# thrill/thrill

Measured on NVIDIA H100. Metric: sort_keys_per_s, higher is better.
Workload: dtype u64

## Files before the change

### thrill_b200/csrc/tg_partition.cuh

```cuda
#pragma once
#include "tg_common.cuh"

namespace tgp {

constexpr int RADIX_BITS = 8;
constexpr int RADIX = 1 << RADIX_BITS;

constexpr u32 FLAG_PARTIAL = 1u << 30;
constexpr u32 FLAG_INCL = 2u << 30;
constexpr u32 VALUE_MASK = (1u << 30) - 1;

template <int WORDS> struct ItemT;
template <> struct ItemT<1> { typedef u64 type; };
template <> struct ItemT<2> { typedef ulonglong2 type; };

__device__ __forceinline__ u64 item_word(const u64& v, int) { return v; }
__device__ __forceinline__ u64 item_word(const ulonglong2& v, int w) { return w ? v.y : v.x; }

struct RadixDigit {
    int word, shift;
    u32 flip;
    static constexpr bool kStoreDigit = false;
    static constexpr bool kHasDrop = false;
    static constexpr int kScratch = 0;
    __device__ __forceinline__ void init() {}
    template <class Item>
    __device__ __forceinline__ u32 operator()(const Item& v, u32) const {
        return ((u32)(item_word(v, word) >> shift) & (RADIX - 1)) ^ flip;
    }
};

__device__ __forceinline__ u32 match_digit8(u32 d) {
    u32 peers;
    asm volatile(
        "{\n"
        ".reg .pred p0, p1, p2, p3, p4, p5, p6, p7;\n"
        ".reg .b32 m0, m1, m2, m3, m4, m5, m6, m7, t;\n"
        "and.b32 t, %1, 1;   setp.ne.u32 p0, t, 0;\n"
        "and.b32 t, %1, 2;   setp.ne.u32 p1, t, 0;\n"
        "and.b32 t, %1, 4;   setp.ne.u32 p2, t, 0;\n"
        "and.b32 t, %1, 8;   setp.ne.u32 p3, t, 0;\n"
        "and.b32 t, %1, 16;  setp.ne.u32 p4, t, 0;\n"
        "and.b32 t, %1, 32;  setp.ne.u32 p5, t, 0;\n"
        "and.b32 t, %1, 64;  setp.ne.u32 p6, t, 0;\n"
        "and.b32 t, %1, 128; setp.ne.u32 p7, t, 0;\n"
        "vote.sync.ballot.b32 m0, p0, 0xffffffff;\n"
        "vote.sync.ballot.b32 m1, p1, 0xffffffff;\n"
        "vote.sync.ballot.b32 m2, p2, 0xffffffff;\n"
        "vote.sync.ballot.b32 m3, p3, 0xffffffff;\n"
        "vote.sync.ballot.b32 m4, p4, 0xffffffff;\n"
        "vote.sync.ballot.b32 m5, p5, 0xffffffff;\n"
        "vote.sync.ballot.b32 m6, p6, 0xffffffff;\n"
        "vote.sync.ballot.b32 m7, p7, 0xffffffff;\n"
        "@!p0 not.b32 m0, m0;\n"
        "@!p1 not.b32 m1, m1;\n"
        "@!p2 not.b32 m2, m2;\n"
        "@!p3 not.b32 m3, m3;\n"
        "@!p4 not.b32 m4, m4;\n"
        "@!p5 not.b32 m5, m5;\n"
        "@!p6 not.b32 m6, m6;\n"
        "@!p7 not.b32 m7, m7;\n"
        "lop3.b32 t, m0, m1, m2, 0x80;\n"
        "lop3.b32 t, t, m3, m4, 0x80;\n"
        "lop3.b32 t, t, m5, m6, 0x80;\n"
        "and.b32 %0, t, m7;\n"
        "}\n"
        : "=r"(peers)
        : "r"(d));
    return peers;
}

constexpr int PEER_MAX = 32;
template <int WORDS, bool STORE = true, bool PEER = false, int SCRATCH = 0>
struct PartCfg {
    static constexpr int THREADS = 512;
    static constexpr int MIN_BLOCKS = 1;
    static constexpr int ITEM_BYTES = 8 * WORDS;
    static constexpr int ITEMS = 32 / WORDS;
    static constexpr int TILE = THREADS * ITEMS;
    static constexpr int HALF = TILE / 2;
    static constexpr int TILE_BYTES = TILE * ITEM_BYTES;
    static constexpr int NWARPS = THREADS / 32;
    static constexpr int BUF_BYTES = TILE_BYTES + (WORDS == 1 ? 16 : 0);
    static constexpr int SMEM = BUF_BYTES + HALF * ITEM_BYTES + NWARPS * RADIX * (int)sizeof(unsigned short) + RADIX * 4 + 64 + 16 + (STORE ? HALF : 0) + (PEER ? PEER_MAX * 8 : 0) + SCRATCH + 128;
    static_assert(SMEM <= 227 * 1024, "partition pass: shared memory of one CTA");
};
constexpr u32 TILE_GROUP = 8;

static __global__ void scan_hist_kernel(const u32* __restrict__ ghist, u32* __restrict__ gbase, u32* __restrict__ skip,
                                 int npass, u32 n) {
    __shared__ u32 warp_tot[RADIX / 32];
    const int d = threadIdx.x;
    for (int p = 0; p < npass; ++p) {
        u32 c = ghist[p * RADIX + d];
        u32 incl = c;
#pragma unroll
        for (int o = 1; o < 32; o <<= 1) {
            u32 t = __shfl_up_sync(0xffffffffu, incl, o);
            if ((d & 31) >= o) incl += t;
        }
        if ((d & 31) == 31) warp_tot[d >> 5] = incl;
        __syncthreads();
        u32 add = 0;
        for (int w = 0; w < (d >> 5); ++w) add += warp_tot[w];
        gbase[p * RADIX + d] = add + incl - c;
        u32 full = __syncthreads_or(c == n);
        if (d == 0 && skip) skip[p] = full ? 1u : 0u;
        __syncthreads();
    }
}

__device__ __forceinline__ u32 lds_u32(u32 addr) {
    u32 v;
    asm volatile("ld.shared.u32 %0, [%1];" : "=r"(v) : "r"(addr) : "memory");
    return v;
}
__device__ __forceinline__ void sts_u32(u32 addr, u32 v) { asm volatile("st.shared.u32 [%0], %1;" ::"r"(addr), "r"(v) : "memory"); }
typedef unsigned short cnt_t;
__device__ __forceinline__ u32 lds_cnt(u32 addr) {
    u32 v;
    asm volatile("ld.shared.u16 %0, [%1];" : "=r"(v) : "r"(addr) : "memory");
    return v;
}
__device__ __forceinline__ void sts_cnt(u32 addr, u32 v) { asm volatile("st.shared.u16 [%0], %1;" ::"r"(addr), "r"(v) : "memory"); }

template <bool FULL, bool STORE, int ITEMS, class Item, class DigitFn>
__device__ __forceinline__ void rank_rows(const Item (&key)[ITEMS], u32 (&rank)[ITEMS], const DigitFn& fn, u32 whist_w,
                                          u32 pos0, u32 tile_base, u32 tile_valid, u32 lt) {
#pragma unroll
    for (int i = 0; i < ITEMS; ++i) {
        const u32 p = pos0 + i * 32;
        u32 d = fn(key[i], tile_base + p);
        if (!FULL && p >= tile_valid) d = RADIX - 1;
        const u32 a = whist_w + d * (u32)sizeof(cnt_t);
        const u32 old = lds_cnt(a);
        const u32 peers = match_digit8(d);
        const u32 below = peers & lt;
        if (below == 0) sts_cnt(a, old + __popc(peers));
        rank[i] = old + __popc(below);
        if (STORE) rank[i] |= d << 16;
        __syncwarp();
    }
}

template <bool STORE, int ITEMS, class Item, class DigitFn>
__device__ __forceinline__ void rank_rows_unstable(const Item (&key)[ITEMS], u32 (&rank)[ITEMS], const DigitFn& fn, u32 whist_w,
                                                   u32 pos0, u32 tile_base) {
#pragma unroll
    for (int i = 0; i < ITEMS; ++i) {
        const u32 d = fn(key[i], tile_base + pos0 + i * 32);
        const u32 sh = (d & 1u) << 4;
        u32 old;
        asm volatile("atom.shared.add.u32 %0, [%1], %2;" : "=r"(old) : "r"(whist_w + (d >> 1) * 4u), "r"(1u << sh) : "memory");
        rank[i] = (old >> sh) & 0xffffu;
        if (STORE) rank[i] |= d << 16;
    }
}

struct SegList {
    const uint4* tiles;
    const u32* segbase;
    u32 num_tiles;
    const u32* num_tiles_dev;
};
__device__ __forceinline__ u32 seg_num_tiles(const SegList& sl) { return sl.num_tiles_dev ? __ldg(sl.num_tiles_dev) : sl.num_tiles; }

template <int WORDS, class DigitFn, bool SEG, bool PEER, bool UNSTABLE>
__global__ void __launch_bounds__(PartCfg<WORDS>::THREADS, PartCfg<WORDS>::MIN_BLOCKS)
partition_kernel(const typename ItemT<WORDS>::type* __restrict__ in, typename ItemT<WORDS>::type* __restrict__ out,
                 u32 n, const DigitFn fn_param, const u32* __restrict__ gbase, u32* __restrict__ status, const SegList sl,
                 typename ItemT<WORDS>::type* const* __restrict__ dbase) {
    typedef typename ItemT<WORDS>::type Item;
    typedef PartCfg<WORDS, DigitFn::kStoreDigit, PEER, DigitFn::kScratch> C;
    constexpr int THREADS = C::THREADS, ITEMS = C::ITEMS, TILE = C::TILE, HALF = C::HALF, NWARPS = C::NWARPS;
    constexpr int LB = 8;
    static_assert(TILE_GROUP <= (u32)LB, "a group member reaches past its group's first tile with one batch");
    static_assert(THREADS >= RADIX, "one thread per digit in the scan phases");

    extern __shared__ __align__(1024) unsigned char smem_raw[];
    Item* const buf = reinterpret_cast<Item*>(smem_raw);
    Item* const xbuf = reinterpret_cast<Item*>(smem_raw + C::BUF_BYTES);
    cnt_t* const whist = reinterpret_cast<cnt_t*>(xbuf + HALF);
    u32* const goff = reinterpret_cast<u32*>(whist + NWARPS * RADIX);
    u32* const warp_tot = goff + RADIX;
    u64* const mbar = reinterpret_cast<u64*>(warp_tot + 16);
    unsigned char* const dig = reinterpret_cast<unsigned char*>(mbar + 2);
    Item** const dptr = reinterpret_cast<Item**>(dig + (DigitFn::kStoreDigit ? HALF : 0));
    unsigned char* const fscratch = reinterpret_cast<unsigned char*>(dptr + (PEER ? PEER_MAX : 0));

    DigitFn fn = fn_param;
    fn.init();
    if constexpr (DigitFn::kScratch > 0) fn.init_shared(fscratch, (int)threadIdx.x, THREADS);
    const int tid = threadIdx.x, lane = tid & 31, warp = tid >> 5;
    const u32 num_tiles = SEG ? seg_num_tiles(sl) : (n + TILE - 1) / TILE;
    const u32 lt = lanemask_lt();
    cnt_t* const whist_w = whist + warp * RADIX;
    const u32 whist_w_a = smem_u32(whist_w);
    const u32 wbase = warp * 32 * ITEMS;

    struct TileInfo { u32 start, len, row, idx, seg; };
    auto tile_info = [&](u32 j) -> TileInfo {
        TileInfo ti;
        if (SEG) {
            const uint4 d = __ldg(&sl.tiles[j]);
            ti.start = d.x; ti.len = d.y; ti.row = d.z; ti.idx = d.w & 0xfffffu; ti.seg = d.w >> 20;
        }
        else {
            ti.start = j * TILE;
            ti.len = (n - ti.start < (u32)TILE) ? n - ti.start : (u32)TILE;
            ti.row = j; ti.idx = j; ti.seg = 0;
        }
        return ti;
    };
    auto tma_shift = [&](const TileInfo& ti) -> u32 { return WORDS == 1 ? (ti.start & 1u) : 0u; };
    auto tma_ok = [&](const TileInfo& ti) -> bool {
        if (ti.len != (u32)TILE) return false;
        return tma_shift(ti) == 0 || (size_t)ti.start + TILE + 1 <= n;
    };

    if (tid == 0) {
        mbar_init(&mbar[0], 1);
        mbar_fence_init();
    }
    if (PEER && tid < PEER_MAX) dptr[tid] = dbase[tid];
    __syncthreads();

    u32 j = blockIdx.x;
    TileInfo tnext = tile_info(j < num_tiles ? j : 0);
    TileInfo tnext2 = tile_info(j + gridDim.x < num_tiles ? j + gridDim.x : 0);
    if (j < num_tiles) {
        const TileInfo t0 = tnext;
        if (tid == 0 && tma_ok(t0)) {
            const u32 sh = tma_shift(t0), bytes = C::TILE_BYTES + 16 * sh;
            mbar_expect_tx(&mbar[0], bytes);
            bulk_g2s(buf, in + (t0.start - sh), bytes, &mbar[0]);
        }
    }
    u32 phase = 0;

    for (; j < num_tiles; j += gridDim.x) {
        const TileInfo ti = tnext;
        if (j + gridDim.x < num_tiles) tnext = tnext2;
        if (SEG ? (j + 2 * gridDim.x < num_tiles) : true) tnext2 = tile_info(j + 2 * gridDim.x);
        const u32 tile_base = ti.start;
        const bool full_tile = ti.len == (u32)TILE;
        const u32 tile_valid = ti.len;
        const bool by_tma = tma_ok(ti);
        const u32* const gb = SEG ? sl.segbase + (size_t)ti.seg * RADIX : gbase;

#pragma unroll
        for (int i = 0; i < RADIX / 64; ++i) reinterpret_cast<u32*>(whist_w)[i * 32 + lane] = 0;

        Item key[ITEMS];
        u32 rank[ITEMS];
        if (by_tma) {
            mbar_wait(&mbar[0], phase);
            phase ^= 1u;
            const Item* src = buf + tma_shift(ti) + wbase + lane;
#pragma unroll
            for (int i = 0; i < ITEMS; ++i) key[i] = src[i * 32];
        }
        else if (full_tile) {
            const Item* src = in + tile_base + wbase + lane;
#pragma unroll
            for (int i = 0; i < ITEMS; ++i) key[i] = src[i * 32];
        }
        else {
#pragma unroll
            for (int i = 0; i < ITEMS; ++i) {
                u32 p = wbase + i * 32 + lane;
                if (p < tile_valid) key[i] = in[(size_t)tile_base + p];
            }
        }
        __syncwarp();

        if (full_tile && UNSTABLE) rank_rows_unstable<DigitFn::kStoreDigit>(key, rank, fn, whist_w_a, wbase + lane, tile_base);
        else if (full_tile) rank_rows<true, DigitFn::kStoreDigit>(key, rank, fn, whist_w_a, wbase + lane, tile_base, tile_valid, lt);
        else rank_rows<false, true>(key, rank, fn, whist_w_a, wbase + lane, tile_base, tile_valid, lt);
        __syncthreads();

        if (tid == 0 && j + gridDim.x < num_tiles) {
            const TileInfo tn = tnext;
            if (tma_ok(tn)) {
                const u32 sh = tma_shift(tn), bytes = C::TILE_BYTES + 16 * sh;
                fence_proxy_async();
                mbar_expect_tx(&mbar[0], bytes);
                bulk_g2s(buf, in + (tn.start - sh), bytes, &mbar[0]);
            }
        }

        u32 count = 0, my_start = 0;
        u32 lbv[SEG ? 1 : LB];
        const u32 my_gb = tid < RADIX ? __ldg(&gb[tid]) : 0u;
        u32* const my_status = status + (size_t)ti.row * RADIX + tid;
        if (tid < RADIX) {
#pragma unroll
            for (int w = 0; w < NWARPS; ++w) count += whist[w * RADIX + tid];
            u32 pub = count;
            if (!full_tile && tid == RADIX - 1) pub -= (u32)TILE - tile_valid;
            st_relaxed_u32(my_status, pub | (ti.idx == 0 ? FLAG_INCL : FLAG_PARTIAL));
            if (SEG) {
                lbv[0] = ti.idx > 0 ? ld_relaxed_u32(my_status - RADIX) : FLAG_INCL;
            }
            else {
#pragma unroll
                for (int k = 0; k < LB; ++k)
                    lbv[k] = ((u32)(k + 1) <= ti.idx) ? ld_relaxed_u32(my_status - (size_t)(k + 1) * RADIX) : FLAG_INCL;
            }
            u32 incl = count;
#pragma unroll
            for (int o = 1; o < 32; o <<= 1) {
                u32 v = __shfl_up_sync(0xffffffffu, incl, o);
                if (lane >= o) incl += v;
            }
            if (lane == 31) warp_tot[warp] = incl;
            my_start = incl - count;
        }
        __syncthreads();
        if (tid < RADIX) {
            for (int w = 0; w < warp; ++w) my_start += warp_tot[w];
            u32 off = my_start;
#pragma unroll
            for (int w = 0; w < NWARPS; ++w) {
                u32 c = whist[w * RADIX + tid];
                whist[w * RADIX + tid] = (cnt_t)off;
                off += c;
            }
        }
        __syncthreads();

#pragma unroll
        for (int r = 0; r < 2; ++r) {
            if (full_tile && !DigitFn::kStoreDigit) {
#pragma unroll
                for (int i = 0; i < ITEMS; ++i) {
                    u32 d = fn(key[i], 0);
                    u32 q = lds_cnt(whist_w_a + d * (u32)sizeof(cnt_t)) + rank[i] - (u32)(r * HALF);
                    if (q < (u32)HALF) xbuf[q] = key[i];
                }
            }
            else {
#pragma unroll
                for (int i = 0; i < ITEMS; ++i) {
                    u32 d = rank[i] >> 16;
                    u32 q = lds_cnt(whist_w_a + d * (u32)sizeof(cnt_t)) + (rank[i] & 0xffffu) - (u32)(r * HALF);
                    if (q < (u32)HALF) {
                        xbuf[q] = key[i];
                        if (DigitFn::kStoreDigit) dig[q] = (unsigned char)d;
                    }
                }
            }

            if (r == 0 && tid < RADIX) {
                u32 excl = 0;
                if (ti.idx > 0) {
                    u32 back = 1;
                    bool done = false;
                    u32 v[LB];
                    if (SEG) {
                        if (lbv[0] & FLAG_INCL) { excl = lbv[0] & VALUE_MASK; done = true; }
                        else {
                            v[0] = lbv[0];
#pragma unroll
                            for (int k = 1; k < LB; ++k)
                                v[k] = (back + k <= ti.idx) ? ld_relaxed_u32(my_status - (size_t)(back + k) * RADIX) : FLAG_INCL;
                        }
                    }
                    else {
#pragma unroll
                        for (int k = 0; k < LB; ++k) v[k] = lbv[k];
                    }
                    while (!done) {
                        bool stalled = false;
#pragma unroll
                        for (int k = 0; k < LB; ++k) {
                            if (!done && !stalled) {
                                if (v[k] & FLAG_INCL) { excl += v[k] & VALUE_MASK; done = true; }
                                else if (v[k] & FLAG_PARTIAL) { excl += v[k] & VALUE_MASK; back++; }
                                else stalled = true;
                            }
                        }
                        if (done) break;
#pragma unroll
                        for (int k = 0; k < LB; ++k)
                            v[k] = (back + k <= ti.idx) ? ld_relaxed_u32(my_status - (size_t)(back + k) * RADIX) : FLAG_INCL;
                    }
                    u32 pub = count;
                    if (!full_tile && tid == RADIX - 1) pub -= (u32)TILE - tile_valid;
                    st_relaxed_u32(my_status, (excl + pub) | FLAG_INCL);
                }
                goff[tid] = my_gb + excl - my_start;
            }
            __syncthreads();

            {
                const Item* const bufp = xbuf + tid;
                const u32 q0 = (u32)(r * HALF) + tid;
                if (full_tile) {
#pragma unroll
                    for (int i = 0; i < HALF / THREADS; ++i) {
                        Item v = bufp[i * THREADS];
                        u32 d = DigitFn::kStoreDigit ? (u32)dig[i * THREADS + tid] : fn(v, 0);
                        if (DigitFn::kHasDrop && d == RADIX - 1) continue;
                        if (PEER) dptr[d][goff[d] + q0 + (u32)(i * THREADS)] = v;
                        else out[goff[d] + q0 + (u32)(i * THREADS)] = v;
                    }
                }
                else {
#pragma unroll
                    for (int i = 0; i < HALF / THREADS; ++i) {
                        if (q0 + (u32)(i * THREADS) < tile_valid) {
                            Item v = bufp[i * THREADS];
                            u32 d = DigitFn::kStoreDigit ? (u32)dig[i * THREADS + tid] : fn(v, 0);
                            if (DigitFn::kHasDrop && d == RADIX - 1) continue;
                            if (PEER) dptr[d][goff[d] + q0 + (u32)(i * THREADS)] = v;
                            else out[goff[d] + q0 + (u32)(i * THREADS)] = v;
                        }
                    }
                }
            }
            __syncthreads();
        }
    }
}

template <int WORDS>
__global__ void copy_items_kernel(const typename ItemT<WORDS>::type* __restrict__ in,
                                  typename ItemT<WORDS>::type* __restrict__ out, size_t n) {
    size_t stride = (size_t)gridDim.x * blockDim.x;
    for (size_t i = (size_t)blockIdx.x * blockDim.x + threadIdx.x; i < n; i += stride) out[i] = in[i];
}

template <int WORDS>
constexpr u32 tile_items() { return (u32)PartCfg<WORDS>::TILE; }
template <int WORDS>
constexpr u32 num_tiles_for(size_t n) { return (u32)((n + tile_items<WORDS>() - 1) / tile_items<WORDS>()); }

template <int WORDS, class DigitFn, bool SEG, bool PEER = false, bool UNSTABLE = false>
int launch_partition_v(tg_ctx* ctx, const void* in, void* out, u32 n, const DigitFn& fn, const u32* gbase, u32* status,
                       const SegList& sl, typename ItemT<WORDS>::type* const* dbase = nullptr) {
    typedef typename ItemT<WORDS>::type Item;
    typedef PartCfg<WORDS, DigitFn::kStoreDigit, PEER, DigitFn::kScratch> C;
    auto kern = partition_kernel<WORDS, DigitFn, SEG, PEER, UNSTABLE>;
    int ctas_per_sm = 0;
    auto it = ctx->kernel_cfg.find((const void*)kern);
    if (it != ctx->kernel_cfg.end()) ctas_per_sm = it->second;
    else {
        TG_CUDA(ctx, cudaFuncSetAttribute(kern, cudaFuncAttributeMaxDynamicSharedMemorySize, C::SMEM));
        TG_CUDA(ctx, cudaOccupancyMaxActiveBlocksPerMultiprocessor(&ctas_per_sm, kern, C::THREADS, C::SMEM));
        if (ctas_per_sm < 1) return tg_set_error(ctx, TG_ERR_CUDA, "partition kernel does not fit on an SM");
        if (ctas_per_sm > C::MIN_BLOCKS) ctas_per_sm = C::MIN_BLOCKS;
        ctx->kernel_cfg[(const void*)kern] = ctas_per_sm;
    }
    u32 num_tiles = SEG ? sl.num_tiles : (n + C::TILE - 1) / C::TILE;
    if (num_tiles == 0) return TG_OK;
    int grid = ctx->sm_count * ctas_per_sm;
    if (grid > (int)num_tiles) grid = (int)num_tiles;
    TG_LAUNCH_T(ctx, TG_K_PARTITION, kern, grid, C::THREADS, C::SMEM, (const Item*)in, (Item*)out, n, fn, gbase, status, sl, dbase);
    return TG_OK;
}

template <int WORDS, class DigitFn>
int launch_partition(tg_ctx* ctx, const void* in, void* out, u32 n, const DigitFn& fn, const u32* gbase, u32* status) {
    return launch_partition_v<WORDS, DigitFn, false>(ctx, in, out, n, fn, gbase, status, SegList{ nullptr, nullptr, 0, nullptr });
}

template <int WORDS, class DigitFn>
int launch_partition_seg(tg_ctx* ctx, const void* in, void* out, u32 n, const DigitFn& fn, u32* status, const SegList& sl) {
    return launch_partition_v<WORDS, DigitFn, true>(ctx, in, out, n, fn, nullptr, status, sl);
}

template <int WORDS, class DigitFn>
int launch_partition_seg_unstable(tg_ctx* ctx, const void* in, void* out, u32 n, const DigitFn& fn, u32* status, const SegList& sl) {
    return launch_partition_v<WORDS, DigitFn, true, false, true>(ctx, in, out, n, fn, nullptr, status, sl);
}

template <int WORDS, class DigitFn>
int launch_partition_peer(tg_ctx* ctx, const void* in, u32 n, const DigitFn& fn, u32* status, const SegList& sl,
                          typename ItemT<WORDS>::type* const* dbase) {
    return launch_partition_v<WORDS, DigitFn, true, true>(ctx, in, nullptr, n, fn, nullptr, status, sl, dbase);
}

}
```

Baseline: 23.89 billion.

## Split partition tile TMA load into four per-stage bulk copies with early refill

The single whole-tile bulk copy into shared memory becomes four stage slots, each with its own mbarrier, and every group of warps waits only on its own quarter. Once all warps of a stage have read their keys, counted through a shared atomic, the last one issues the next tile's copy for that slot right away instead of waiting for the post-ranking __syncthreads. Partial and unaligned tiles now also go through bulk copies, with granule padding and a fallback global read at the tail. This aims to overlap the next tile's load with ranking and the scatter, at the cost of more barriers, atomics and edge-case complexity.

```diff
diff --git a/thrill_b200/csrc/tg_partition.cuh b/thrill_b200/csrc/tg_partition.cuh
--- a/thrill_b200/csrc/tg_partition.cuh
+++ b/thrill_b200/csrc/tg_partition.cuh
@@ -81,8 +81,14 @@
     static constexpr int HALF = TILE / 2;
     static constexpr int TILE_BYTES = TILE * ITEM_BYTES;
     static constexpr int NWARPS = THREADS / 32;
-    static constexpr int BUF_BYTES = TILE_BYTES + (WORDS == 1 ? 16 : 0);
-    static constexpr int SMEM = BUF_BYTES + HALF * ITEM_BYTES + NWARPS * RADIX * (int)sizeof(unsigned short) + RADIX * 4 + 64 + 16 + (STORE ? HALF : 0) + (PEER ? PEER_MAX * 8 : 0) + SCRATCH + 128;
+    static constexpr int STAGES = 4;
+    static constexpr int STAGE_WARPS = NWARPS / STAGES;
+    static constexpr int STAGE_ITEMS = TILE / STAGES;
+    static constexpr int GRANULE = 16 / ITEM_BYTES;
+    static constexpr int SLOT = STAGE_ITEMS + (GRANULE > 1 ? GRANULE : 0);
+    static constexpr int BUF_BYTES = STAGES * SLOT * ITEM_BYTES;
+    static constexpr int SMEM = BUF_BYTES + HALF * ITEM_BYTES + NWARPS * RADIX * (int)sizeof(unsigned short) + RADIX * 4 + 64 + STAGES * 12 + (STORE ? HALF : 0) + (PEER ? PEER_MAX * 8 : 0) + SCRATCH + 128;
+    static_assert(NWARPS % STAGES == 0 && STAGE_ITEMS % GRANULE == 0, "partition pass: a stage is whole warps and granules");
     static_assert(SMEM <= 227 * 1024, "partition pass: shared memory of one CTA");
 };
 constexpr u32 TILE_GROUP = 8;
@@ -184,7 +190,8 @@
     u32* const goff = reinterpret_cast<u32*>(whist + NWARPS * RADIX);
     u32* const warp_tot = goff + RADIX;
     u64* const mbar = reinterpret_cast<u64*>(warp_tot + 16);
-    unsigned char* const dig = reinterpret_cast<unsigned char*>(mbar + 2);
+    u32* const sread = reinterpret_cast<u32*>(mbar + C::STAGES);
+    unsigned char* const dig = reinterpret_cast<unsigned char*>(sread + C::STAGES);
     Item** const dptr = reinterpret_cast<Item**>(dig + (DigitFn::kStoreDigit ? HALF : 0));
     unsigned char* const fscratch = reinterpret_cast<unsigned char*>(dptr + (PEER ? PEER_MAX : 0));
 
@@ -198,28 +205,52 @@
     const u32 whist_w_a = smem_u32(whist_w);
     const u32 wbase = warp * 32 * ITEMS;
 
-    struct TileInfo { u32 start, len, row, idx, seg; };
+    struct TileInfo {
+        u32 start, len, row, w;
+        __device__ __forceinline__ u32 idx() const { return w & 0xfffffu; }
+        __device__ __forceinline__ u32 seg() const { return w >> 20; }
+    };
     auto tile_info = [&](u32 j) -> TileInfo {
         TileInfo ti;
         if (SEG) {
             const uint4 d = __ldg(&sl.tiles[j]);
-            ti.start = d.x; ti.len = d.y; ti.row = d.z; ti.idx = d.w & 0xfffffu; ti.seg = d.w >> 20;
+            ti.start = d.x; ti.len = d.y; ti.row = d.z; ti.w = d.w;
         }
         else {
             ti.start = j * TILE;
             ti.len = (n - ti.start < (u32)TILE) ? n - ti.start : (u32)TILE;
-            ti.row = j; ti.idx = j; ti.seg = 0;
+            ti.row = j; ti.w = j;
         }
         return ti;
     };
     auto tma_shift = [&](const TileInfo& ti) -> u32 { return WORDS == 1 ? (ti.start & 1u) : 0u; };
-    auto tma_ok = [&](const TileInfo& ti) -> bool {
-        if (ti.len != (u32)TILE) return false;
-        return tma_shift(ti) == 0 || (size_t)ti.start + TILE + 1 <= n;
+    struct Span { u32 src, end; };
+    auto stage_span = [&](const TileInfo& ti, u32 s) -> Span {
+        Span sp;
+        sp.src = ti.start + s * (u32)C::STAGE_ITEMS - tma_shift(ti);
+        sp.end = sp.src;
+        if (s * (u32)C::STAGE_ITEMS < ti.len) {
+            const u32 last = ti.start + min((s + 1) * (u32)C::STAGE_ITEMS, ti.len);
+            constexpr u32 GR = (u32)C::GRANULE;
+            sp.end = min((last + GR - 1) / GR * GR, n / GR * GR);
+        }
+        return sp;
     };
+    auto start_copy = [&](const TileInfo& ti, u32 s) {
+        const Span sp = stage_span(ti, s);
+        if (sp.end > sp.src) {
+            const u32 bytes = (sp.end - sp.src) * (u32)C::ITEM_BYTES;
+            mbar_expect_tx(&mbar[s], bytes);
+            bulk_g2s(buf + s * C::SLOT, in + sp.src, bytes, &mbar[s]);
+        }
+    };
 
     if (tid == 0) {
-        mbar_init(&mbar[0], 1);
+#pragma unroll
+        for (int s = 0; s < C::STAGES; ++s) {
+            mbar_init(&mbar[s], 1);
+            sread[s] = 0;
+        }
         mbar_fence_init();
     }
     if (PEER && tid < PEER_MAX) dptr[tid] = dbase[tid];
@@ -228,14 +259,11 @@
     u32 j = blockIdx.x;
     TileInfo tnext = tile_info(j < num_tiles ? j : 0);
     TileInfo tnext2 = tile_info(j + gridDim.x < num_tiles ? j + gridDim.x : 0);
-    if (j < num_tiles) {
-        const TileInfo t0 = tnext;
-        if (tid == 0 && tma_ok(t0)) {
-            const u32 sh = tma_shift(t0), bytes = C::TILE_BYTES + 16 * sh;
-            mbar_expect_tx(&mbar[0], bytes);
-            bulk_g2s(buf, in + (t0.start - sh), bytes, &mbar[0]);
-        }
-    }
+    if (j < num_tiles && tid == 0) {
+#pragma unroll
+        for (int s = 0; s < C::STAGES; ++s) start_copy(tnext, (u32)s);
+    }
+    const u32 stage = (u32)warp / (u32)C::STAGE_WARPS;
     u32 phase = 0;
 
     for (; j < num_tiles; j += gridDim.x) {
@@ -245,49 +273,47 @@
         const u32 tile_base = ti.start;
         const bool full_tile = ti.len == (u32)TILE;
         const u32 tile_valid = ti.len;
-        const bool by_tma = tma_ok(ti);
-        const u32* const gb = SEG ? sl.segbase + (size_t)ti.seg * RADIX : gbase;
+        const u32* const gb = SEG ? sl.segbase + (size_t)ti.seg() * RADIX : gbase;
 
 #pragma unroll
         for (int i = 0; i < RADIX / 64; ++i) reinterpret_cast<u32*>(whist_w)[i * 32 + lane] = 0;
 
         Item key[ITEMS];
         u32 rank[ITEMS];
-        if (by_tma) {
-            mbar_wait(&mbar[0], phase);
-            phase ^= 1u;
-            const Item* src = buf + tma_shift(ti) + wbase + lane;
-#pragma unroll
-            for (int i = 0; i < ITEMS; ++i) key[i] = src[i * 32];
-        }
-        else if (full_tile) {
-            const Item* src = in + tile_base + wbase + lane;
-#pragma unroll
-            for (int i = 0; i < ITEMS; ++i) key[i] = src[i * 32];
-        }
-        else {
-#pragma unroll
-            for (int i = 0; i < ITEMS; ++i) {
-                u32 p = wbase + i * 32 + lane;
-                if (p < tile_valid) key[i] = in[(size_t)tile_base + p];
+        {
+            const Span sp = stage_span(ti, stage);
+            if (sp.end > sp.src) {
+                mbar_wait(&mbar[stage], phase);
+                phase ^= 1u;
+            }
+            Item* const tile_buf = buf + stage * (C::SLOT - C::STAGE_ITEMS) + tma_shift(ti);
+            if (tile_base + min(wbase + 32 * ITEMS, tile_valid) <= sp.end) {
+#pragma unroll
+                for (int i = 0; i < ITEMS; ++i) key[i] = tile_buf[wbase + lane + i * 32];
+            }
+            else {
+#pragma unroll
+                for (int i = 0; i < ITEMS; ++i) {
+                    const u32 p = wbase + i * 32 + lane;
+                    if (tile_base + p < sp.end) key[i] = tile_buf[p];
+                    else if (p < tile_valid) key[i] = in[n - 1];
+                }
             }
         }
         __syncwarp();
+        if (lane == 0) {
+            u32 before;
+            asm volatile("atom.acq_rel.cta.shared::cta.add.u32 %0, [%1], 1;" : "=r"(before) : "r"(smem_u32(&sread[stage])) : "memory");
+            if (before % (u32)C::STAGE_WARPS == (u32)C::STAGE_WARPS - 1 && j + gridDim.x < num_tiles) {
+                fence_proxy_async();
+                start_copy(tnext, stage);
+            }
+        }
 
         if (full_tile && UNSTABLE) rank_rows_unstable<DigitFn::kStoreDigit>(key, rank, fn, whist_w_a, wbase + lane, tile_base);
         else if (full_tile) rank_rows<true, DigitFn::kStoreDigit>(key, rank, fn, whist_w_a, wbase + lane, tile_base, tile_valid, lt);
         else rank_rows<false, true>(key, rank, fn, whist_w_a, wbase + lane, tile_base, tile_valid, lt);
         __syncthreads();
-
-        if (tid == 0 && j + gridDim.x < num_tiles) {
-            const TileInfo tn = tnext;
-            if (tma_ok(tn)) {
-                const u32 sh = tma_shift(tn), bytes = C::TILE_BYTES + 16 * sh;
-                fence_proxy_async();
-                mbar_expect_tx(&mbar[0], bytes);
-                bulk_g2s(buf, in + (tn.start - sh), bytes, &mbar[0]);
-            }
-        }
 
         u32 count = 0, my_start = 0;
         u32 lbv[SEG ? 1 : LB];
@@ -298,14 +324,14 @@
             for (int w = 0; w < NWARPS; ++w) count += whist[w * RADIX + tid];
             u32 pub = count;
             if (!full_tile && tid == RADIX - 1) pub -= (u32)TILE - tile_valid;
-            st_relaxed_u32(my_status, pub | (ti.idx == 0 ? FLAG_INCL : FLAG_PARTIAL));
+            st_relaxed_u32(my_status, pub | (ti.idx() == 0 ? FLAG_INCL : FLAG_PARTIAL));
             if (SEG) {
-                lbv[0] = ti.idx > 0 ? ld_relaxed_u32(my_status - RADIX) : FLAG_INCL;
+                lbv[0] = ti.idx() > 0 ? ld_relaxed_u32(my_status - RADIX) : FLAG_INCL;
             }
             else {
 #pragma unroll
                 for (int k = 0; k < LB; ++k)
-                    lbv[k] = ((u32)(k + 1) <= ti.idx) ? ld_relaxed_u32(my_status - (size_t)(k + 1) * RADIX) : FLAG_INCL;
+                    lbv[k] = ((u32)(k + 1) <= ti.idx()) ? ld_relaxed_u32(my_status - (size_t)(k + 1) * RADIX) : FLAG_INCL;
             }
             u32 incl = count;
 #pragma unroll
@@ -353,7 +379,7 @@
 
             if (r == 0 && tid < RADIX) {
                 u32 excl = 0;
-                if (ti.idx > 0) {
+                if (ti.idx() > 0) {
                     u32 back = 1;
                     bool done = false;
                     u32 v[LB];
@@ -363,7 +389,7 @@
                             v[0] = lbv[0];
 #pragma unroll
                             for (int k = 1; k < LB; ++k)
-                                v[k] = (back + k <= ti.idx) ? ld_relaxed_u32(my_status - (size_t)(back + k) * RADIX) : FLAG_INCL;
+                                v[k] = (back + k <= ti.idx()) ? ld_relaxed_u32(my_status - (size_t)(back + k) * RADIX) : FLAG_INCL;
                         }
                     }
                     else {
@@ -383,7 +409,7 @@
                         if (done) break;
 #pragma unroll
                         for (int k = 0; k < LB; ++k)
-                            v[k] = (back + k <= ti.idx) ? ld_relaxed_u32(my_status - (size_t)(back + k) * RADIX) : FLAG_INCL;
+                            v[k] = (back + k <= ti.idx()) ? ld_relaxed_u32(my_status - (size_t)(back + k) * RADIX) : FLAG_INCL;
                     }
                     u32 pub = count;
                     if (!full_tile && tid == RADIX - 1) pub -= (u32)TILE - tile_valid;
```

Result: faster. 24.18 billion (median of 6 runs) (+1.2%).
